# SamsungSAILMontreal/ghn3

Measured on AMD Instinct MI355X. Metric: predicted-params/sec (GHN fwd+bwd), ghn3xlm16, 256-node graphs, higher is better.
Workload: dtype f16; 1 GPU; ghn3xlm16 fwd+bwd, 1 synthetic 256-node graph(s) per GPU (seed 256000+), 86515016 predicted params per GPU, loss = sum of Frobenius norms of the predicted tensors; ghn_params=654365312, decoder_rows=1421, workspace_bytes=2436048640, zero_fill_bytes=2797339192, parallelism=dp1, index_mode=reference, loss=fused into the tile kernels

## Files before the change

ghn3_amd/csrc/elementwise.hip:

```cpp

#include "ghn3_internal.h"

#define MAX_DEGREE 100
#define MAX_INPUT_DIST 1000

__device__ __forceinline__ float wsum(float v) {
#pragma unroll
    for (int o = 32; o > 0; o >>= 1) v += __shfl_xor(v, o, 64);
    return v;
}

static int launch_ok(const char* what) {
    hipError_t e = hipGetLastError();
    if (e != hipSuccess) { ghn3_set_error("%s launch: %s", what, hipGetErrorString(e)); return GHN3_E_HIP; }
    return GHN3_OK;
}

__global__ __launch_bounds__(256) void graph_prologue_kernel(const int64_t* __restrict__ A, int* __restrict__ deg_in,
                                                             int* __restrict__ deg_out, int* __restrict__ dist0,
                                                             int* __restrict__ pair, int N, int V) {
    __shared__ int red[2][4];
    const int i = blockIdx.x, b = blockIdx.y;
    const int64_t* Ab = A + (size_t)b * N * N;
    int cnt_out = 0, cnt_in = 0;
    for (int j = threadIdx.x; j < N; j += 256) {
        const int64_t fw = Ab[(size_t)i * N + j];
        const int64_t bw = Ab[(size_t)j * N + i];
        cnt_out += (fw == 1);
        cnt_in += (bw == 1);
        int f = (int)(fw < 0 ? 0 : (fw >= V ? V - 1 : fw));
        int g = (int)(bw < 0 ? 0 : (bw >= V ? V - 1 : bw));
        pair[((size_t)b * N + i) * N + j] = f * V + g;
    }
#pragma unroll
    for (int o = 32; o > 0; o >>= 1) {
        cnt_out += __shfl_xor(cnt_out, o, 64);
        cnt_in += __shfl_xor(cnt_in, o, 64);
    }
    const int w = threadIdx.x >> 6;
    if ((threadIdx.x & 63) == 0) { red[0][w] = cnt_out; red[1][w] = cnt_in; }
    __syncthreads();
    if (threadIdx.x == 0) {
        int o_ = red[0][0] + red[0][1] + red[0][2] + red[0][3];
        int i_ = red[1][0] + red[1][1] + red[1][2] + red[1][3];
        deg_out[b * N + i] = o_ > MAX_DEGREE ? MAX_DEGREE : o_;
        deg_in[b * N + i] = i_ > MAX_DEGREE ? MAX_DEGREE : i_;
        int64_t dd = Ab[i];
        dist0[b * N + i] = (int)(dd < 0 ? 0 : (dd > MAX_INPUT_DIST ? MAX_INPUT_DIST : dd));
    }
}

int ghn3_graph_prologue(const int64_t* A, int* deg_in, int* deg_out, int* dist0, int* pair, int B, int N, int V,
                        hipStream_t s) {
    hipLaunchKernelGGL(graph_prologue_kernel, dim3(N, B), dim3(256), 0, s, A, deg_in, deg_out, dist0, pair, N, V);
    return launch_ok("graph_prologue");
}

__global__ __launch_bounds__(256) void embed_nodes_kernel(
    float* __restrict__ x, const int* __restrict__ node_type, const int* __restrict__ shape_idx,
    const int* __restrict__ n_nodes, const int* __restrict__ node_off, const float* __restrict__ E_type,
    const float* __restrict__ E_ch, const float* __restrict__ E_sp, const float* __restrict__ E_in,
    const float* __restrict__ E_out, const float* __restrict__ E_dist, const int* __restrict__ deg_in,
    const int* __restrict__ deg_out, const int* __restrict__ dist0, int B, int N, int C) {
    const int row = blockIdx.x * 4 + (threadIdx.x >> 6);
    if (row >= B * N) return;
    const int lane = threadIdx.x & 63;
    const int b = row / N, i = row - b * N;
    float* xr = x + (size_t)row * C;
    if (i >= n_nodes[b]) {
        for (int c = lane; c < C; c += 64) xr[c] = 0.f;
        return;
    }
    const int sidx = node_off[b] + i;
    const int t = node_type[sidx];
    const int s0 = shape_idx[4 * sidx], s1 = shape_idx[4 * sidx + 1], s2 = shape_idx[4 * sidx + 2],
              s3 = shape_idx[4 * sidx + 3];
    const int di = deg_in[row], dout = deg_out[row], dd = dist0[row];
    const int cq = C >> 2;
    for (int c = lane; c < C; c += 64) {
        const int part = c / cq, cc = c - part * cq;
        float sh;
        if (part == 0) sh = E_ch[(size_t)s0 * cq + cc];
        else if (part == 1) sh = E_ch[(size_t)s1 * cq + cc];
        else if (part == 2) sh = E_sp[(size_t)s2 * cq + cc];
        else sh = E_sp[(size_t)s3 * cq + cc];
        float v = E_type[(size_t)t * C + c] + sh;
        v += E_in[(size_t)di * C + c];
        v += E_out[(size_t)dout * C + c];
        v += E_dist[(size_t)dd * C + c];
        xr[c] = v;
    }
}

int ghn3_embed_nodes(float* x, const int* node_type, const int* shape_idx, const int* n_nodes, const int* node_off,
                     const float* E_type, const float* E_ch, const float* E_sp, const float* E_in,
                     const float* E_out, const float* E_dist, const int* deg_in, const int* deg_out,
                     const int* dist0, int B, int N, int C, hipStream_t s) {
    if (C % 4) { ghn3_set_error("embed: C=%d not a multiple of 4", C); return GHN3_E_ARG; }
    hipLaunchKernelGGL(embed_nodes_kernel, dim3((B * N + 3) / 4), dim3(256), 0, s, x, node_type, shape_idx, n_nodes,
                       node_off, E_type, E_ch, E_sp, E_in, E_out, E_dist, deg_in, deg_out, dist0, B, N, C);
    return launch_ok("embed_nodes");
}

__global__ __launch_bounds__(256) void embed_bwd_kernel(
    const float* __restrict__ dx, const int* __restrict__ node_type, const int* __restrict__ shape_idx,
    const int* __restrict__ n_nodes, const int* __restrict__ node_off, float* __restrict__ dE_type,
    float* __restrict__ dE_ch, float* __restrict__ dE_sp, float* __restrict__ dE_in, float* __restrict__ dE_out,
    float* __restrict__ dE_dist, const int* __restrict__ deg_in, const int* __restrict__ deg_out,
    const int* __restrict__ dist0, int B, int N, int C, int n_type, int n_ch, int n_sp) {
    extern __shared__ unsigned long long emb_mask[];
    int r = blockIdx.x, tab = 0;
    if (r >= n_type) { r -= n_type; tab = 1;
        if (r >= n_ch) { r -= n_ch; tab = 2;
            if (r >= n_sp) { r -= n_sp; tab = 3;
                if (r >= 101) { r -= 101; tab = 4;
                    if (r >= 101) { r -= 101; tab = 5; } } } } }
    const int cq = C >> 2;
    const int width = (tab == 1 || tab == 2) ? cq : C;
    const int base0 = tab == 2 ? 2 * cq : 0, base1 = tab == 1 ? cq : 3 * cq;
    const int rows = B * N, words = (rows + 63) >> 6;
    int any = 0;
    for (int row0 = (threadIdx.x >> 6) * 64; row0 < rows; row0 += 256) {
        const int row = row0 + (threadIdx.x & 63);
        int f = 0;
        if (row < rows) {
            const int b = row / N, i = row - b * N;
            if (i < n_nodes[b]) {
                const int sidx = node_off[b] + i;
                if (tab == 0) f = node_type[sidx] == r;
                else if (tab == 1) f = (shape_idx[4 * sidx] == r) | ((shape_idx[4 * sidx + 1] == r) << 1);
                else if (tab == 2) f = (shape_idx[4 * sidx + 2] == r) | ((shape_idx[4 * sidx + 3] == r) << 1);
                else if (tab == 3) f = deg_in[row] == r;
                else if (tab == 4) f = deg_out[row] == r;
                else f = dist0[row] == r;
            }
        }
        const unsigned long long m0 = __ballot(f & 1), m1 = __ballot(f & 2);
        if ((threadIdx.x & 63) == 0) { emb_mask[row0 >> 6] = m0; emb_mask[words + (row0 >> 6)] = m1; }
        any |= f;
    }
    if (!__syncthreads_or(any)) return;
    int* lst = reinterpret_cast<int*>(emb_mask + 2 * words);
    __shared__ int n_match;
    if (threadIdx.x == 0) {
        int n = 0;
        for (int w = 0; w < words; ++w) {
            const unsigned long long m0 = emb_mask[w], m1 = emb_mask[words + w];
            unsigned long long m = m0 | m1;
            while (m) {
                const int bit = __ffsll((long long)m) - 1;
                m &= m - 1;
                lst[n++] = (w * 64 + bit) | ((int)((m0 >> bit) & 1) << 24) | ((int)((m1 >> bit) & 1) << 25);
            }
        }
        n_match = n;
    }
    __syncthreads();
    const int n = n_match;
    float acc[2] = {0.f, 0.f};
    for (int i0 = 0; i0 < n; i0 += 8) {
        float v0[8][2], v1[8][2];
#pragma unroll
        for (int e = 0; e < 8; ++e) {
            const int ent = i0 + e < n ? lst[i0 + e] : 0;
            const float* g = dx + (size_t)(ent & 0xffffff) * C;
#pragma unroll
            for (int k = 0; k < 2; ++k) {
                const int c = threadIdx.x + 256 * k;
                const bool in = i0 + e < n && c < width;
                v0[e][k] = (in && (ent & (1 << 24))) ? g[base0 + c] : 0.f;
                v1[e][k] = (in && (ent & (1 << 25))) ? g[base1 + c] : 0.f;
            }
        }
#pragma unroll
        for (int e = 0; e < 8; ++e)
#pragma unroll
            for (int k = 0; k < 2; ++k) { acc[k] += v0[e][k]; acc[k] += v1[e][k]; }
    }
    float* dst = tab == 0 ? dE_type : tab == 1 ? dE_ch : tab == 2 ? dE_sp : tab == 3 ? dE_in : tab == 4 ? dE_out : dE_dist;
#pragma unroll
    for (int k = 0; k < 2; ++k) {
        const int c = threadIdx.x + 256 * k;
        if (c < width) dst[(size_t)r * width + c] += acc[k];
    }
}

int ghn3_embed_bwd(const float* dx, const int* node_type, const int* shape_idx, const int* n_nodes,
                   const int* node_off, float* dE_type, float* dE_ch, float* dE_sp, float* dE_in, float* dE_out,
                   float* dE_dist, const int* deg_in, const int* deg_out, const int* dist0, int B, int N, int C,
                   int n_type, int n_ch, int n_sp, hipStream_t s) {
    if (C > 512 || n_type <= 0 || n_ch <= 0 || n_sp <= 0) {
        ghn3_set_error("embed_bwd: C <= 512 and the table row counts (i3..i5) are required");
        return GHN3_E_ARG;
    }
    if (B * N > 12 * 1024) { ghn3_set_error("embed_bwd: more than 12288 dense node rows"); return GHN3_E_LIMIT; }
    const int blocks = n_type + n_ch + n_sp + 101 + 101 + 1001;
    hipLaunchKernelGGL(embed_bwd_kernel, dim3(blocks), dim3(256), (size_t)(16 * ((B * N + 63) / 64) + 4 * (size_t)B * N + 16), s, dx, node_type, shape_idx, n_nodes,
                       node_off, dE_type, dE_ch, dE_sp, dE_in, dE_out, dE_dist, deg_in, deg_out, dist0, B, N, C, n_type,
                       n_ch, n_sp);
    return launch_ok("embed_bwd");
}

__global__ __launch_bounds__(256) void edge_hidden_kernel(float* __restrict__ hid, const float* __restrict__ Pfw,
                                                          const float* __restrict__ Pbw, int V, int C) {
    const int p = blockIdx.x;
    const int fw = p / V, bw = p - fw * V;
    for (int c = threadIdx.x; c < C; c += 256)
        hid[(size_t)p * C + c] = fmaxf(Pfw[(size_t)fw * C + c] + Pbw[(size_t)bw * C + c], 0.f);
}
int ghn3_edge_hidden(float* hid, const float* Pfw, const float* Pbw, int V, int C, hipStream_t s) {
    hipLaunchKernelGGL(edge_hidden_kernel, dim3(V * V), dim3(256), 0, s, hid, Pfw, Pbw, V, C);
    return launch_ok("edge_hidden");
}

__global__ __launch_bounds__(256) void edge_hidden_bwd_fw_kernel(float* __restrict__ dPfw, float* __restrict__ dhid,
                                                                 const float* __restrict__ hid, int V, int C) {
    __shared__ float part[4][64];
    const int fw = blockIdx.x, c = blockIdx.y * 64 + (threadIdx.x & 63), w = threadIdx.x >> 6;
    float acc = 0.f;
    if (c < C)
        for (int bw = w; bw < V; bw += 4) {
            const size_t o = ((size_t)fw * V + bw) * C + c;
            const float g = hid[o] > 0.f ? dhid[o] : 0.f;
            dhid[o] = g;
            acc += g;
        }
    part[w][threadIdx.x & 63] = acc;
    __syncthreads();
    if (w == 0 && c < C) dPfw[(size_t)fw * C + c] = (part[0][threadIdx.x] + part[1][threadIdx.x]) + (part[2][threadIdx.x] + part[3][threadIdx.x]);
}
__global__ __launch_bounds__(256) void edge_hidden_bwd_bw_kernel(float* __restrict__ dPbw,
                                                                 const float* __restrict__ dhid, int V, int C) {
    __shared__ float part[4][64];
    const int bw = blockIdx.x, c = blockIdx.y * 64 + (threadIdx.x & 63), w = threadIdx.x >> 6;
    float acc = 0.f;
    if (c < C)
        for (int fw = w; fw < V; fw += 4) acc += dhid[((size_t)fw * V + bw) * C + c];
    part[w][threadIdx.x & 63] = acc;
    __syncthreads();
    if (w == 0 && c < C) dPbw[(size_t)bw * C + c] = (part[0][threadIdx.x] + part[1][threadIdx.x]) + (part[2][threadIdx.x] + part[3][threadIdx.x]);
}
int ghn3_edge_hidden_bwd(float* dPfw, float* dPbw, float* dhid, const float* hid, int V, int C, hipStream_t s) {
    hipLaunchKernelGGL(edge_hidden_bwd_fw_kernel, dim3(V, (C + 63) / 64), dim3(256), 0, s, dPfw, dhid, hid, V, C);
    hipLaunchKernelGGL(edge_hidden_bwd_bw_kernel, dim3(V, (C + 63) / 64), dim3(256), 0, s, dPbw, dhid, V, C);
    return launch_ok("edge_hidden_bwd");
}

__global__ __launch_bounds__(256) void bias_gather_kernel(float* __restrict__ bias, const float* __restrict__ T,
                                                          const int* __restrict__ pair, int N, int H, int ldT) {
    extern __shared__ float bg_rows[];
    __shared__ int bg_pair[256];
    const int b = blockIdx.z, i = blockIdx.y;
    const int j0 = blockIdx.x * 256, j = j0 + threadIdx.x;
    const int nj = min(256, N - j0);
    bg_pair[threadIdx.x] = j < N ? pair[((size_t)b * N + i) * N + j] : 0;
    __syncthreads();
    const int lpr = ldT >> 2;
    const int ld = ldT + 1;
    for (int e = threadIdx.x; e < nj * lpr; e += 256) {
        const int q = e / lpr, c = e - q * lpr;
        const float4 v = *reinterpret_cast<const float4*>(T + (size_t)bg_pair[q] * ldT + 4 * c);
        float* d = bg_rows + q * ld + 4 * c;
        d[0] = v.x; d[1] = v.y; d[2] = v.z; d[3] = v.w;
    }
    __syncthreads();
    if (j >= N) return;
    const float* r = bg_rows + threadIdx.x * ld;
    for (int h = 0; h < H; ++h) bias[(((size_t)b * H + h) * N + i) * N + j] = r[h];
}
__global__ __launch_bounds__(256) void bias_gather_direct_kernel(float* __restrict__ bias, const float* __restrict__ T,
                                                                 const int* __restrict__ pair, int N, int H, int ldT) {
    const int b = blockIdx.z, i = blockIdx.y;
    const int j = blockIdx.x * 256 + threadIdx.x;
    if (j >= N) return;
    const int p = pair[((size_t)b * N + i) * N + j];
    const float* tr = T + (size_t)p * ldT;
    for (int h = 0; h < H; ++h) bias[(((size_t)b * H + h) * N + i) * N + j] = tr[h];
}
int ghn3_bias_gather(float* bias, const float* T, const int* pair, int B, int N, int H, hipStream_t s) {
    const int ldT = (H + 3) & ~3;
    if (ldT <= 64)
        hipLaunchKernelGGL(bias_gather_kernel, dim3((N + 255) / 256, N, B), dim3(256), 256 * (ldT + 1) * sizeof(float), s, bias, T,
                           pair, N, H, ldT);
    else
        hipLaunchKernelGGL(bias_gather_direct_kernel, dim3((N + 255) / 256, N, B), dim3(256), 0, s, bias, T, pair, N, H, ldT);
    return launch_ok("bias_gather");
}

__global__ __launch_bounds__(256) void bias_amax_kernel(const float* __restrict__ x, int64_t n, float* __restrict__ amax) {
    float m = 0.f;
    const int64_t n4 = (reinterpret_cast<uintptr_t>(x) & 15) ? 0 : (n >> 2);
    const float4* x4 = reinterpret_cast<const float4*>(x);
    for (int64_t e = (int64_t)blockIdx.x * 256 + threadIdx.x; e < n4; e += (int64_t)gridDim.x * 256) {
        const float4 v = x4[e];
        m = fmaxf(fmaxf(m, fmaxf(fabsf(v.x), fabsf(v.y))), fmaxf(fabsf(v.z), fabsf(v.w)));
    }
    for (int64_t e = 4 * n4 + (int64_t)blockIdx.x * 256 + threadIdx.x; e < n; e += (int64_t)gridDim.x * 256) m = fmaxf(m, fabsf(x[e]));
    ghn3_atomic_amax(amax, m);
}
__device__ __forceinline__ float fix_scale(float amax) {
    if (!(amax > 0.f)) return 1.f;
    const int e = (int)((__float_as_uint(amax) >> 23) & 0xff) - 127;
    return __uint_as_float((unsigned)(127 + 30 - e) << 23);
}
__global__ __launch_bounds__(256) void bias_hist_kernel(long long* __restrict__ acc, const float* __restrict__ dBias,
                                                        const int* __restrict__ pair, int N, int H, int V,
                                                        int rows_per_block, int use_lds, const float* __restrict__ amax) {
    extern __shared__ __attribute__((aligned(16))) long long hist[];
    const int b = blockIdx.z, h = blockIdx.y;
    const int i0 = blockIdx.x * rows_per_block;
    const int i1 = min(N, i0 + rows_per_block);
    const int bins = V * V;
    const float sc = fix_scale(*amax);
    if (use_lds) {
        for (int k = threadIdx.x; k < bins; k += 256) hist[k] = 0;
        __syncthreads();
    }
    const size_t total = (size_t)(i1 - i0) * N;
    for (size_t e = threadIdx.x; e < total; e += 256) {
        const size_t off = (size_t)i0 * N + e;
        const int p = pair[(size_t)b * N * N + off];
        const long long g = (long long)llrintf(dBias[((size_t)b * H + h) * N * N + off] * sc);
        if (g == 0) continue;
        if (use_lds) atomicAdd(reinterpret_cast<unsigned long long*>(&hist[p]), (unsigned long long)g);
        else atomicAdd(reinterpret_cast<unsigned long long*>(&acc[(size_t)p * H + h]), (unsigned long long)g);
    }
    if (use_lds) {
        __syncthreads();
        for (int k = threadIdx.x; k < bins; k += 256) {
            const long long v = hist[k];
            if (v != 0) atomicAdd(reinterpret_cast<unsigned long long*>(&acc[(size_t)k * H + h]), (unsigned long long)v);
        }
    }
}
__global__ __launch_bounds__(256) void bias_hist_finish_kernel(float* __restrict__ dT, const long long* __restrict__ acc,
                                                               int bins, int H, int ldT, const float* __restrict__ amax) {
// ... 1663 lines not shown
```

ghn3_amd/csrc/gemm_wg.hip:

```cpp

#include "ghn3_internal.h"

#define GAS __attribute__((address_space(1)))
typedef float f32x4 __attribute__((ext_vector_type(4)));
typedef __bf16 bf16x8 __attribute__((ext_vector_type(8)));
typedef f32x4 GAS* gf4;
typedef const f32x4 GAS* gcf4;

namespace {

constexpr int WG_KC = 64;
template <int T> constexpr int wg_lds() { return 4 * T * 128 + 16 * T * 4; }

__device__ __forceinline__ unsigned wg_pack(__bf16 a, __bf16 b) {
    return (unsigned)__builtin_bit_cast(unsigned short, a) | ((unsigned)__builtin_bit_cast(unsigned short, b) << 16);
}

__device__ __forceinline__ void wg_stage(char* s_hi, char* s_lo, int f, int k, const f32x4& r0, const f32x4& r1) {
#pragma unroll
    for (int e = 0; e < 4; ++e) {
        const __bf16 h0 = (__bf16)r0[e], h1 = (__bf16)r1[e];
        const __bf16 l0 = (__bf16)(r0[e] - (float)h0), l1 = (__bf16)(r1[e] - (float)h1);
        const int row = f + e;
        const int off = row * 128 + (((k >> 3) ^ ((row >> 1) & 7)) << 4) + ((k & 7) << 1);
        *reinterpret_cast<unsigned*>(s_hi + off) = wg_pack(h0, h1);
        *reinterpret_cast<unsigned*>(s_lo + off) = wg_pack(l0, l1);
    }
}

template <int T>
__device__ __forceinline__ void wg_tile(const GemmProbDev* __restrict__ probs, int n_probs, int tile, char* sm) {
    constexpr int WG_BM = T, WG_BN = T;
    constexpr int TN = T / 32;
    constexpr int FPR = T / 4;
    char* sAh = sm;
    char* sAl = sm + T * 128;
    char* sBh = sm + 2 * T * 128;
    char* sBl = sm + 3 * T * 128;
    float* sbias = reinterpret_cast<float*>(sm + 4 * T * 128);

    int lo = 0, hi_ = n_probs - 1;
    while (lo < hi_) {
        const int mid = (lo + hi_ + 1) >> 1;
        if (probs[mid].tile_start <= tile) lo = mid; else hi_ = mid - 1;
    }
    const GemmProbDev* P = probs + lo;
    const int t_id = tile - P->tile_start;
    const int n0 = (t_id % P->tiles_n) * WG_BN, m0 = (t_id / P->tiles_n) * WG_BM;
    const int M = P->M, N = P->N, K = P->K, lda = P->lda, ldb = P->ldb;
    const int tid = threadIdx.x, lane = tid & 63, wave = tid >> 6;
    const int l15 = lane & 15, lq = lane >> 4;
    const int wm0 = (wave >> 1) * 32, wn0 = (wave & 1) * (T / 2);
    const bool want_bias = (P->flags & GHN3_GEMM_BIASGRAD) && n0 == 0;

    constexpr int FGW = FPR / 8;
    const int f4 = ((lane & 7) + 8 * (wave % FGW)) * 4, kp = (lane >> 3) + 8 * (wave / FGW);
    const float GAS* Ag = (const float GAS*)P->A;
    const float GAS* Bg = (const float GAS*)P->B;
    const bool a_in = m0 + f4 < M, b_in = n0 + f4 < N;
    const f32x4 zero = f32x4{0.f, 0.f, 0.f, 0.f};

    f32x4 ra[2][2], rb[2][2];
    auto load_chunk = [&](int k0) {
#pragma unroll
        for (int i = 0; i < 2; ++i)
#pragma unroll
            for (int r = 0; r < 2; ++r) {
                const int k = k0 + 2 * kp + 32 * i + r;
                ra[i][r] = (a_in && k < K) ? *reinterpret_cast<gcf4>(Ag + (int64_t)k * lda + m0 + f4) : zero;
                rb[i][r] = (b_in && k < K) ? *reinterpret_cast<gcf4>(Bg + (int64_t)k * ldb + n0 + f4) : zero;
            }
    };

    f32x4 acc0[2][TN], acc1[2][TN];
#pragma unroll
    for (int i = 0; i < 2; ++i)
#pragma unroll
        for (int j = 0; j < TN; ++j) { acc0[i][j] = zero; acc1[i][j] = zero; }
    f32x4 bsum = zero;

    load_chunk(0);
    for (int k0 = 0; k0 < K; k0 += WG_KC) {
        if (k0 > 0) __syncthreads();
#pragma unroll
        for (int i = 0; i < 2; ++i) {
            wg_stage(sAh, sAl, f4, 2 * kp + 32 * i, ra[i][0], ra[i][1]);
            wg_stage(sBh, sBl, f4, 2 * kp + 32 * i, rb[i][0], rb[i][1]);
            if (want_bias) bsum += ra[i][0] + ra[i][1];
        }
        if (k0 + WG_KC < K) load_chunk(k0 + WG_KC);
        __syncthreads();
#pragma unroll
        for (int h = 0; h < 2; ++h) {
            const int ch = 4 * h + lq;
            bf16x8 xh[2], xl[2], wh[TN], wl[TN];
#pragma unroll
            for (int i = 0; i < 2; ++i) {
                const int row = wm0 + 16 * i + l15;
                const int off = row * 128 + ((ch ^ ((row >> 1) & 7)) << 4);
                xh[i] = *reinterpret_cast<const bf16x8*>(sAh + off);
                xl[i] = *reinterpret_cast<const bf16x8*>(sAl + off);
            }
#pragma unroll
            for (int j = 0; j < TN; ++j) {
                const int row = wn0 + 16 * j + l15;
                const int off = row * 128 + ((ch ^ ((row >> 1) & 7)) << 4);
                wh[j] = *reinterpret_cast<const bf16x8*>(sBh + off);
                wl[j] = *reinterpret_cast<const bf16x8*>(sBl + off);
            }
#pragma unroll
            for (int i = 0; i < 2; ++i)
#pragma unroll
                for (int j = 0; j < TN; ++j) {
                    acc0[i][j] = __builtin_amdgcn_mfma_f32_16x16x32_bf16(wh[j], xh[i], acc0[i][j], 0, 0, 0);
                    acc1[i][j] = __builtin_amdgcn_mfma_f32_16x16x32_bf16(wh[j], xl[i], acc1[i][j], 0, 0, 0);
                }
#pragma unroll
            for (int i = 0; i < 2; ++i)
#pragma unroll
                for (int j = 0; j < TN; ++j)
                    acc1[i][j] = __builtin_amdgcn_mfma_f32_16x16x32_bf16(wl[j], xh[i], acc1[i][j], 0, 0, 0);
        }
    }

    const float alpha = P->alpha;
    const bool accum = (P->flags & GHN3_GEMM_ACCUM) != 0;
    float GAS* C = (float GAS*)P->C;
#pragma unroll
    for (int i = 0; i < 2; ++i) {
        const int m = m0 + wm0 + 16 * i + l15;
#pragma unroll
        for (int j = 0; j < TN; ++j) {
            const int n = n0 + wn0 + 16 * j + 4 * lq;
            if (m >= M || n >= N) continue;
            const int64_t ci = (int64_t)m * P->ldc + n;
            f32x4 v;
#pragma unroll
            for (int e = 0; e < 4; ++e) v[e] = (acc0[i][j][e] + acc1[i][j][e]) * alpha;
            if (accum) v += *reinterpret_cast<gcf4>(C + ci);
            *reinterpret_cast<gf4>(C + ci) = v;
        }
    }
    if (want_bias) {
#pragma unroll
        for (int e = 0; e < 4; ++e) sbias[kp * T + f4 + e] = bsum[e];
        __syncthreads();
        if (tid < T && m0 + tid < M) {
            float t = 0.f;
#pragma unroll
            for (int q = 0; q < 16; ++q) t += sbias[q * T + tid];
            float GAS* db = (float GAS*)P->bias + (int64_t)(m0 + tid) * P->bias_stride;
            *db += t;
        }
    }
}

template <int T>
__global__ __launch_bounds__(T * 4) void gemm_wg_kernel(const GemmProbDev* __restrict__ probs, int n_probs, int total_tiles) {
    extern __shared__ __attribute__((aligned(16))) char wg_sm[];
    for (int tile = blockIdx.x; tile < total_tiles; tile += gridDim.x) {
        wg_tile<T>(probs, n_probs, tile, wg_sm);
        __syncthreads();
    }
}

}

int ghn3_gemm_wg_launch(const GemmProbDev* d_probs, int n_probs, int total_tiles, int grid_cap, int tile_edge, hipStream_t stream) {
    if (n_probs <= 0 || total_tiles <= 0) return GHN3_OK;
    const int grid = grid_cap > 0 && grid_cap < total_tiles ? grid_cap : total_tiles;
    if (tile_edge == 128) {
        static bool attr = false;
        if (!attr) {
            hipFuncSetAttribute((const void*)gemm_wg_kernel<128>, hipFuncAttributeMaxDynamicSharedMemorySize, wg_lds<128>());
            attr = true;
        }
        hipLaunchKernelGGL(gemm_wg_kernel<128>, dim3(grid), dim3(512), wg_lds<128>(), stream, d_probs, n_probs, total_tiles);
    } else {
        hipLaunchKernelGGL(gemm_wg_kernel<64>, dim3(grid), dim3(256), wg_lds<64>(), stream, d_probs, n_probs, total_tiles);
    }
    hipError_t e = hipGetLastError();
    if (e != hipSuccess) { ghn3_set_error("wgrad x3 gemm launch: %s", hipGetErrorString(e)); return GHN3_E_HIP; }
    return GHN3_OK;
}
```

ghn3_amd/program.py:

```python

import math
import os

import numpy as np

from . import _lib as L
from . import bookkeeping as bk

ALIGN = 256


def global_param_names():
    return ['ln.weight', 'ln.bias', 'embed.weight', 'shape_enc.embed_spatial.weight',
            'shape_enc.embed_channel.weight', 'gnn.0.centrality_embed_in.weight',
            'gnn.0.centrality_embed_out.weight', 'gnn.0.input_dist_embed.weight',
            'gnn.0.attn.edge_embed.embed.weight', 'gnn.0.attn.proj_e.0.weight', 'gnn.0.attn.proj_e.0.bias',
            'gnn.0.attn.proj_e.2.weight', 'gnn.0.attn.proj_e.2.bias',
            'decoder.fc.0.weight', 'decoder.fc.0.bias', 'decoder.conv.0.weight', 'decoder.conv.0.bias',
            'decoder.conv.2.weight', 'decoder.conv.2.bias', 'decoder.class_layer_predictor.1.weight',
            'decoder.class_layer_predictor.1.bias', 'decoder_1d.fc.0.weight', 'decoder_1d.fc.0.bias',
            'decoder_1d.fc.2.weight', 'decoder_1d.fc.2.bias', 'bias_class.1.weight', 'bias_class.1.bias']


LAYER_PARAM_NAMES = ['ln1.weight', 'ln1.bias', 'attn.to_qkv.weight', 'attn.to_out.0.weight', 'attn.to_out.0.bias',
# ... 1161 lines not shown
                                scale)
                            predicted[-1]['tok'] = (tok_off, i_e)
                            tok_off += round_up(i_e, 4)
                        else:
                            raise NotImplementedError('1-D target from a 4-D tile')
                    elif len(key) == 2 and key[1] > 0:
                        g, n_idx = group_of[ind]
                        base = g['cls_off'][n_idx]
                        if len(t) == 4 and (t[2], t[3]) != (1, 1):
                            raise NotImplementedError('classifier target %s' % str(t))
                        add(dst, 1, base, (t[0], t[1], 1, 1), (min(t[0], K), min(t[1], g['i']), 1, 1),
                            (1, ldK, 0, 0), (K, g['i'], 1, 1), mode, scale)
                    elif len(key) == 2 and key[1] < 0:
                        r = clsb_row[ind]
                        assert len(t) == 1
                        add(dst, 3, r * ldK, (1, t[0], 1, 1), (1, min(t[0], K), 1, 1), (0, 1, 0, 0), (1, K, 1, 1),
                            mode, scale)
                    else:
                        r = self.oned_index[ind]
                        if len(t) == 1:
                            half = (1 - int(bool(is_w)) + it)
                            add(dst, 2, r * 2 * mc + half * mc, (1, t[0], 1, 1), (1, min(t[0], mc), 1, 1),
                                (0, 1, 0, 0), (1, mc, 1, 1), mode, scale)
                        elif len(t) == 3:
                            if t[1] > 1 and t[2] > 1:
                                raise NotImplementedError('3-D target %s from the 1-D decoder' % str(t))
                            add(dst, 2, r * 2 * mc, (t[0], t[1], t[2], 1), (min(t[0], 2 * mc), 1, 1, 1),
                                (1, 0, 0, 0), (2 * mc, 1, 1, 1), mode, scale)
                        else:
                            raise NotImplementedError('target %s from the 1-D decoder' % str(t))
        self.predicted = predicted
        self.out_numel = max(out_off, 16)
        self.tok_floats = max(tok_off, 4)
        self.n_desc = nd = len(descs)
        CH = 2048
        self.tile_lds = [0, 0]
        desc_arr = np.zeros(max(nd, 1), dtype=L.TILE_DT)
        fb = bb = np.zeros((0, 2), dtype=np.int64)
        if nd:
            cols = list(zip(*descs))
            desc_arr['dst_off'], desc_arr['src_off'] = cols[0], cols[1]
            S = np.asarray(cols[2], dtype=np.int64).reshape(nd, 4)
            T = np.asarray(cols[3], dtype=np.int64).reshape(nd, 4)
            E = np.asarray(cols[4], dtype=np.int64).reshape(nd, 4)
            R = np.asarray(cols[5], dtype=np.int64).reshape(nd, 4)
            desc_arr['S'], desc_arr['T'], desc_arr['E'], desc_arr['R'] = S, T, E, R
            desc_arr['src_buf'], desc_arr['mode'], desc_arr['scale'] = cols[6], cols[7], cols[8]
            mode = np.asarray(cols[7], dtype=np.int64)
            hw = T[:, 2] * T[:, 3]
            row_ok = (mode == 0) & (hw > 1) & (S[:, 1] == 1) & (E[:, 2] == T[:, 2]) & (T[:, 2] == R[:, 2]) & \
                (E[:, 3] == T[:, 3]) & (T[:, 3] == R[:, 3]) & (hw <= 1024)
            ich = np.maximum(16, np.minimum(np.maximum(T[:, 1], R[:, 1]), (4096 // np.maximum(hw, 1)) // 16 * 16))
            desc_arr['_pad'] = np.where(row_ok, ich, 0)
            if row_ok.any():
                lds = int((4 * ich * hw)[row_ok].max())
                self.tile_lds = [lds, lds]
            ids = np.arange(nd, dtype=np.int64)

            def tables(n0, n1, numel):
                n_i = (n1 + ich - 1) // ich
                cnt = np.where(row_ok, n0 * n_i, (numel + CH - 1) // CH)
                total = int(cnt.sum())
                first = np.cumsum(cnt) - cnt
                d_of = np.repeat(ids, cnt)
                j = np.arange(total, dtype=np.int64) - np.repeat(first, cnt)
                rb = row_ok[d_of]
                ni_b = np.maximum(n_i[d_of], 1)
                word = np.where(rb, (j // ni_b) | (((j % ni_b) * ich[d_of]) << 24), j * CH)
                return np.stack([np.where(rb, ~d_of, d_of), word], axis=1), first

            fb, fwd_first = tables(T[:, 0], T[:, 1], T.prod(axis=1))
            bb, _ = tables(R[:, 0], R[:, 1], R.prod(axis=1))
        dseg = np.asarray(desc_seg if nd else [0], dtype=np.int32)
        raw = np.concatenate([desc_arr.view(np.uint8).reshape(-1), fb.view(np.uint8).reshape(-1),
                              bb.view(np.uint8).reshape(-1), dseg.view(np.uint8).reshape(-1)])
        self.r_desc = self.idx(raw)
        self.fwd_blk = (len(fb), desc_arr.nbytes)
        self.bwd_blk = (len(bb), desc_arr.nbytes + fb.nbytes)
        self.desc_seg_off = desc_arr.nbytes + fb.nbytes + bb.nbytes
        seg_blk = np.zeros(len(predicted) + 1, dtype=np.int32)
        if nd:
            first_desc = np.full(len(predicted), nd, dtype=np.int64)
            np.minimum.at(first_desc, dseg, np.arange(nd))
            seg_blk[:-1] = fwd_first[first_desc]
        seg_blk[-1] = len(fb)
        self.r_seg_blk = self.idx(seg_blk)
        seg = np.asarray([[p['offset'], p['offset'] + p['numel']] for p in predicted], dtype=np.int64).reshape(-1, 2)
        self.r_seg = self.idx(seg if len(seg) else np.zeros((1, 2), dtype=np.int64))
        self.n_seg = len(predicted)
        ends = seg[:, 1] if len(seg) else np.zeros(1, dtype=np.int64)
        starts = np.arange(0, max(self.out_numel, 1), 8192, dtype=np.int64)
        self.r_seg_first = self.idx(np.searchsorted(ends, starts, side='right').astype(np.int32))
        srcs = self._tile_sources(False)
        if self.n_desc:
            parts = self.wsf('sq_parts', self.fwd_blk[0]) if self.training else self.NONE
            bparts = self.wsf('b_parts', self.fwd_blk[0]) if self.training else self.NONE
            self._tile_desc_arr = desc_arr
            self.op(L.OP_TILE_FWD, refs=[(self.xbuf(self.X_OUT), 0)] + srcs + [self.r_desc, parts, bparts],
                    ints=(self.n_desc, self.fwd_blk[0], self.fwd_blk[1], self.tile_lds[0]),
                    flags=L.OPFLAG_TIMED | (self.TAG_TILE_FWD << 16))

    def _tile_sources(self, grad):
        pre = 'd_' if grad else ''
        out = []
        for name in ('tiles', 'clsout', 'w1d', 'cbout'):
            nm = pre + name
            out.append(self.wref(nm) if nm in self._ws_names else self.NONE)
        if grad:
            out.append(self.wsf('d_tok', self.tok_floats))
        else:
            out.append((self.xbuf(self.X_TOK), 0))
        out.append(self.NONE)
        return out

    def norm_ops(self, upstream=1.0):
        scal = self.xbuf(self.X_SCAL)
        f_ops, b_ops = [], []
        saved = self._ops
        self._ops = []
        self.op(L.OP_MEMSET0, refs=((scal, 0),), ints=(4,))
        self.op(L.OP_PARAM_NORM_FWD, refs=((scal, 0), (self.xbuf(self.X_OUT), 0), self.r_seg, (scal, 256),
                                           self.r_seg_first, (scal, 256 + round_up(4 * max(self.n_seg, 1), 64))),
                ints=(self.n_seg, self.out_numel))
        f_ops = self._finish_ops()
        self.op(L.OP_PARAM_NORM_BWD, refs=((self.xbuf(self.X_DOUT), 0), (self.xbuf(self.X_OUT), 0), self.r_seg,
                                           (scal, 256), self.r_seg_first), ints=(self.n_seg, self.out_numel),
                floats=(upstream,))
        b_ops = self._finish_ops()
        self._ops = saved
        return f_ops, b_ops

    def norm_fin_ops(self):
        scal = self.xbuf(self.X_SCAL)
        saved, self._ops = self._ops, []
        if self.n_desc and 'sq_parts' in self._ws_names:
            self.op(L.OP_PARAM_NORM_FIN, refs=((scal, 0), (scal, 256), self.wref('sq_parts'), self.r_seg_blk,
                                               self.wref('b_parts'), (scal, 256 + round_up(4 * max(self.n_seg, 1), 64)),
                                               (scal, 252)),
                    ints=(self.n_seg,))
        else:
            self.op(L.OP_MEMSET0, refs=((scal, 0),), ints=(4,))
        ops = self._finish_ops()
        self._ops = saved
        return ops

    def _layer_side_ops(self, layers, rows):
        C = self.C
        p0 = len(self._probs)
        for d in layers:
            pre = d['pre']
            W3, W1f, Wo, Wq = pre + 'ff.net.3.weight', pre + 'ff.net.0.weight', pre + 'attn.to_out.0.weight', \
                pre + 'attn.to_qkv.weight'
            self.gemm(d['g_cur'], d['f'], self.gref(W3), C, 4 * C, rows, C, 4 * C, 4 * C, a_mode=L.MODE_COL,
                      b_mode=L.MODE_COL, accum=True, dbias=self.gref(pre + 'ff.net.3.bias'))
            self.gemm(d['dz'], d['h2'], self.gref(W1f), 4 * C, C, rows, 4 * C, C, C, a_mode=L.MODE_COL, b_mode=L.MODE_COL,
                      accum=True, dbias=self.gref(pre + 'ff.net.0.bias'))
            self.gemm(d['g_mid'], d['o'], self.gref(Wo), C, C, rows, C, C, C, a_mode=L.MODE_COL, b_mode=L.MODE_COL,
                      accum=True, dbias=self.gref(pre + 'attn.to_out.0.bias'))
            self.gemm(d['dqkv'], d['h1'], self.gref(Wq), 3 * C, C, rows, 3 * C, C, C, a_mode=L.MODE_COL, b_mode=L.MODE_COL,
                      accum=True)
        dflt = ('48' if self.x3 else '64') if C >= 256 else '0'
        self.gemm_op(p0, side=True, tile=int(os.environ.get('GHN3_LAYER_WGRAD_TILE', dflt)),
                     grid_cap=int(os.environ.get('GHN3_LAYER_WGRAD_CAP', '0')) if self.SIDE else 0)
        if len(layers) == 1:
            d = layers[0]
            pre = d['pre']
            self.op(L.OP_LN_PARAM_GRAD, refs=(self.gref(pre + 'ln2.weight'), self.gref(pre + 'ln2.bias'), d['dhA'], d['xmid'],
                                              d['m2'], d['r2']), ints=(rows, C, 1), flags=self.SIDE)
            self.op(L.OP_LN_PARAM_GRAD, refs=(self.gref(pre + 'ln1.weight'), self.gref(pre + 'ln1.bias'), d['dhB'], d['x_in'],
                                              d['m1'], d['r1']), ints=(rows, C, 1), flags=self.SIDE)
            return
        base = 'gnn.0.' + LAYER_PARAM_NAMES[0]
        ws = self.xbuf(self.X_WS)
        tab = []
        for d in layers:
            pre = d['pre']
            for (gn, bn, dy, x, mu, rs) in ((pre + 'ln2.weight', pre + 'ln2.bias', d['dhA'], d['xmid'], d['m2'], d['r2']),
                                           (pre + 'ln1.weight', pre + 'ln1.bias', d['dhB'], d['x_in'], d['m1'], d['r1'])):
                assert all(r_[0] == ws and r_[1] % 4 == 0 for r_ in (dy, x, mu, rs))
                tab.append((self.param_gap(base, gn), self.param_gap(base, bn), dy[1] // 4, x[1] // 4, mu[1] // 4, rs[1] // 4))
        self.op(L.OP_LN_PARAM_GRAD_BATCH, refs=(self.gref(base), (ws, 0), self.idx(np.asarray(tab, dtype=np.int64))),
                ints=(len(tab), rows, C), flags=self.SIDE)

    def _colsum(self, out, X, M, N, ld, q=0, s=0, stride=1, gather=None):
        self.op(L.OP_COLSUM, refs=(out, X, gather if gather is not None else self.NONE),
                ints=(M, N, ld, q, s, stride, 1))

    def set_tile_route(self, direct):
        direct = bool(direct and getattr(self, 'tile_bwd_h16', 0))
        if self.tile_bwd_op is None or not hasattr(self, 'd16_kinds'):
            return []
        self.bwd_ops[self.tile_bwd_op]['i'][5] = self.tile_bwd_h16 if direct else 0
        touched = []
        for idx, on in ((self.d16_on_idx, direct), (self.d16_off_idx, not direct)):
            for k in idx:
                self.bwd_ops[k]['kind'] = self.d16_kinds[k] if on else L.OP_NOP
                touched.append(k)
        return touched

    @staticmethod
    def _wgrad_order_env():
        return os.environ.get('GHN3_WGRAD_ORDER', 'first' if os.environ.get('GHN3_WGRAD_LATE', '1') != '0' else 'early')

    def _wgrad_schedule(self, flops, rows):
        env_main, env_cap = os.environ.get('GHN3_WGRAD_MAIN'), os.environ.get('GHN3_WGRAD_CAP')
        if not self.SIDE or env_main == '1':
            return 0
        if env_cap is not None:
            return max(8, int(env_cap) // 8 * 8)
        w_ms = flops / 1150e12 * 1e3 + 4.0 * self.max_shape[0] * self.max_shape[1] * 8 * self.C / 4.3e12 * 1e3
        ch_ms = self.Lyr * (0.030 + 0.014 * (rows / 256.0) * (self.C / 384.0) ** 2)
        if env_main != '0' and w_ms < 0.75 * ch_ms:
            return 0
        if self._wgrad_order_env() == 'first':
            return 128
        c = int(round(256.0 * w_ms / (1.75 * ch_ms) / 8.0)) * 8
        if c >= 232:
            return 0 if env_main != '0' else 224
        return max(64, c)

    def _build_h16_table(self, g16, direct_member):
        D = self._tile_desc_arr
        nd = self.n_desc
        tab = np.zeros((nd, 3), dtype=np.int64)
        tab[:, 0] = np.iinfo(np.int64).min
        members = []
        for g in g16:
            for m_ in g['members']:
                if direct_member(m_):
                    members.append((m_['tile_off'], m_['tile_off'] + m_['rows'] * g['ld'], g))
        members.sort(key=lambda t: t[0])
        if members and nd:
            lo = np.asarray([t[0] for t in members], dtype=np.int64)
            hi = np.asarray([t[1] for t in members], dtype=np.int64)
            src = D['src_off'].astype(np.int64)
            k = np.searchsorted(lo, src, side='right') - 1
            ok = (D['src_buf'] == 0) & (k >= 0)
            ok &= src < hi[np.maximum(k, 0)]
            reach = src + ((D['R'].astype(np.int64) - 1) * D['S'].astype(np.int64)).sum(axis=1)
            d_tiles_h = self._ws_names['d_tiles'] // 2
            for d_ in np.nonzero(ok)[0]:
                g = members[int(k[d_])][2]
                assert reach[d_] < hi[int(k[d_])], 'tile descriptor straddles a family member'
                assert D['mode'][d_] == 0
                rel0 = int(src[d_]) - g['tile_off']
                assert 0 <= rel0 and g['rows'] * g['ld'] < 2 ** 32
                tab[d_] = (g['dth'] - d_tiles_h, rel0, g['ld'] | (g['dth_ld'] << 32))
        r_tab = self.idx(tab)
        assert r_tab[0] == self.r_desc[0] and r_tab[1] > self.r_desc[1]
        self.tile_bwd_h16 = r_tab[1] - self.r_desc[1]

    def _build_backward(self):
        C, H, B, N, V, K = self.C, self.H, self.B, self.N, self.V, self.K
        rows = B * N
        ldT, ldK = self.ldT, self.ldK
        ms = self.max_shape
        S2 = self.S * self.S
        M, n1 = self.M, self.n1
        (r_types, r_shape, r_nn, r_noff, deg_in, deg_out, dist0, pair) = self.r_graph
        xe = self.r_xe
        self.op(L.OP_MEMSET0, refs=((self.xbuf(self.X_GRADFLAT), 0),), ints=(-1,))
        self.op(L.OP_MEMSET0, refs=((self.xbuf(self.X_GRADFLAT), 0),), ints=(-1,))
        self.memset_grad_op = 0
        self.tile_bwd_op = None
        self.grad_no_memset = []
        self.bwd_cut_w2 = 0
        late_ops = []
        self.wgrad_op_range = None
        self.grad_sumsq = None

        d_rows = self.wsf('d_xrows', (M + n1) * C)
        zeros = []
        if M > 0:
            self.wsf('d_tiles', self.tiles_floats)
            self.ws_zero_dout = [(self._ws_names['d_tiles'], 4 * (int(self.tiles_floats) + 64))]
            if 'clsout' in self._ws_names:
                n_cls = sum(g['rows'] * g['i_ld'] for g in self.conv_groups if g['kind'] == 'cls')
                self.wsf('d_clsout', n_cls * ldK)
                zeros.append((self.wref('d_clsout'), 4 * n_cls * ldK))
        if n1 > 0:
            mc = self.mc
            self.wsf('d_w1d', n1 * 2 * mc)
            zeros.append((self.wref('d_w1d'), 4 * n1 * 2 * mc))
            if self.n1_clsb:
                self.wsf('d_cbout', self.n1_clsb * ldK)
                zeros.append((self.wref('d_cbout'), 4 * self.n1_clsb * ldK))
        self.r_amax = self.wsf('amax', 16)
        scaled = self.bwd_scaled and self.direct16 and M > 0
        amax_t = self.r_amax if scaled else None
        amax_u = (self.r_amax[0], self.r_amax[1] + 16) if scaled else None
        if scaled:
            zeros.append((self.r_amax, 64))
        run = None
        for (buf, off), n in sorted(zeros, key=lambda it: (it[0][0], it[0][1])) + [((None, 0), 0)]:
            if run is not None and buf == run[0] and 0 <= off - (run[1] + run[2]) <= 1024:
                run[2] = off + n - run[1]
                continue
            if run is not None:
                self.op(L.OP_MEMSET0, refs=((run[0], run[1]),), ints=(run[2],))
            run = [buf, off, n]
        if self.n_desc:
            grads = self._tile_sources(True)
            if scaled:
                grads[5] = amax_t
            srcs = self._tile_sources(False)
            self.tile_bwd_op = len(self._ops)
            self.tile_bwd_refs = {0: (self.xbuf(self.X_DOUT), 0), 6: (self.xbuf(self.X_NORMG), 0),
                                  14: (self.xbuf(self.X_SCAL), 256), 15: (self.xbuf(self.X_OUT), 0)}
            self.op(L.OP_TILE_BWD, refs=[(self.xbuf(self.X_DOUT), 0)] + srcs + [self.r_desc] + grads +
                    [self.NONE, self.NONE],
                    ints=(self.n_desc, self.bwd_blk[0], self.bwd_blk[1], self.tile_lds[1], self.desc_seg_off, 0,
                          1 if self.decoder_bwd_ctype == L.CT_BF16 else 0),
                    flags=L.OPFLAG_TIMED | (self.TAG_TILE_BWD << 16))
# ... 541 lines not shown
```

Baseline: 15.04 billion predicted-params/s.

## Parallelize embed backward across waves and transpose-read LDS in weight-grad GEMM

The embedding backward kernel now builds its match list with all four waves using popcount prefix sums, then splits the summation across waves and reduces the partials in shared memory. This replaces the single-thread list build and the serial per-block sum. The weight-gradient GEMM switches to a k-major LDS layout that is staged with vector bf16 conversions and read through ds_read_tr16 transpose loads. It also prefetches the old C values at tile start and adds a waves_per_eu occupancy hint. The layer weight-gradient GEMMs drop accumulate mode, which removes the read of C but assumes those gradient buffers are not already holding values that must be added to.

```diff
diff --git a/ghn3_amd/csrc/elementwise.hip b/ghn3_amd/csrc/elementwise.hip
--- a/ghn3_amd/csrc/elementwise.hip
+++ b/ghn3_amd/csrc/elementwise.hip
@@ -102,6 +102,30 @@
     return launch_ok("embed_nodes");
 }
 
+template <int NJ, int E, bool TWO>
+__device__ __forceinline__ void embed_bwd_sum(const float* __restrict__ dx, const int* lst, int begin, int end, int C,
+                                              int width, int base0, int base1, int lane, float* acc) {
+    for (int i0 = begin; i0 < end; i0 += E) {
+        float v0[E][NJ], v1[E][NJ];
+#pragma unroll
+        for (int e = 0; e < E; ++e) {
+            const int ent = i0 + e < end ? lst[i0 + e] : 0;
+            const float* g = dx + (size_t)(ent & 0xffffff) * C;
+#pragma unroll
+            for (int j = 0; j < NJ; ++j) {
+                const int c = lane + 64 * j;
+                const bool in = i0 + e < end && c < width;
+                v0[e][j] = (in && (ent & (1 << 24))) ? g[base0 + c] : 0.f;
+                v1[e][j] = (TWO && in && (ent & (1 << 25))) ? g[base1 + c] : 0.f;
+            }
+        }
+#pragma unroll
+        for (int e = 0; e < E; ++e)
+#pragma unroll
+            for (int j = 0; j < NJ; ++j) { acc[j] += v0[e][j]; if (TWO) acc[j] += v1[e][j]; }
+    }
+}
+
 __global__ __launch_bounds__(256) void embed_bwd_kernel(
     const float* __restrict__ dx, const int* __restrict__ node_type, const int* __restrict__ shape_idx,
     const int* __restrict__ n_nodes, const int* __restrict__ node_off, float* __restrict__ dE_type,
@@ -109,6 +133,7 @@
     float* __restrict__ dE_dist, const int* __restrict__ deg_in, const int* __restrict__ deg_out,
     const int* __restrict__ dist0, int B, int N, int C, int n_type, int n_ch, int n_sp) {
     extern __shared__ unsigned long long emb_mask[];
+    __shared__ float part[4][512];
     int r = blockIdx.x, tab = 0;
     if (r >= n_type) { r -= n_type; tab = 1;
         if (r >= n_ch) { r -= n_ch; tab = 2;
@@ -119,9 +144,10 @@
     const int width = (tab == 1 || tab == 2) ? cq : C;
     const int base0 = tab == 2 ? 2 * cq : 0, base1 = tab == 1 ? cq : 3 * cq;
     const int rows = B * N, words = (rows + 63) >> 6;
+    const int lane = threadIdx.x & 63, wave = threadIdx.x >> 6;
     int any = 0;
-    for (int row0 = (threadIdx.x >> 6) * 64; row0 < rows; row0 += 256) {
-        const int row = row0 + (threadIdx.x & 63);
+    for (int row0 = wave * 64; row0 < rows; row0 += 256) {
+        const int row = row0 + lane;
         int f = 0;
         if (row < rows) {
             const int b = row / N, i = row - b * N;
@@ -136,52 +162,32 @@
             }
         }
         const unsigned long long m0 = __ballot(f & 1), m1 = __ballot(f & 2);
-        if ((threadIdx.x & 63) == 0) { emb_mask[row0 >> 6] = m0; emb_mask[words + (row0 >> 6)] = m1; }
+        if (lane == 0) { emb_mask[row0 >> 6] = m0; emb_mask[words + (row0 >> 6)] = m1; }
         any |= f;
     }
     if (!__syncthreads_or(any)) return;
     int* lst = reinterpret_cast<int*>(emb_mask + 2 * words);
-    __shared__ int n_match;
-    if (threadIdx.x == 0) {
-        int n = 0;
-        for (int w = 0; w < words; ++w) {
-            const unsigned long long m0 = emb_mask[w], m1 = emb_mask[words + w];
-            unsigned long long m = m0 | m1;
-            while (m) {
-                const int bit = __ffsll((long long)m) - 1;
-                m &= m - 1;
-                lst[n++] = (w * 64 + bit) | ((int)((m0 >> bit) & 1) << 24) | ((int)((m1 >> bit) & 1) << 25);
-            }
-        }
-        n_match = n;
-    }
-    __syncthreads();
-    const int n = n_match;
-    float acc[2] = {0.f, 0.f};
-    for (int i0 = 0; i0 < n; i0 += 8) {
-        float v0[8][2], v1[8][2];
-#pragma unroll
-        for (int e = 0; e < 8; ++e) {
-            const int ent = i0 + e < n ? lst[i0 + e] : 0;
-            const float* g = dx + (size_t)(ent & 0xffffff) * C;
-#pragma unroll
-            for (int k = 0; k < 2; ++k) {
-                const int c = threadIdx.x + 256 * k;
-                const bool in = i0 + e < n && c < width;
-                v0[e][k] = (in && (ent & (1 << 24))) ? g[base0 + c] : 0.f;
-                v1[e][k] = (in && (ent & (1 << 25))) ? g[base1 + c] : 0.f;
-            }
-        }
-#pragma unroll
-        for (int e = 0; e < 8; ++e)
-#pragma unroll
-            for (int k = 0; k < 2; ++k) { acc[k] += v0[e][k]; acc[k] += v1[e][k]; }
-    }
+    int n = 0;
+    for (int w = 0; w < words; ++w) {
+        const unsigned long long m0 = emb_mask[w], m1 = emb_mask[words + w], m = m0 | m1;
+        if ((w & 3) == wave && ((m >> lane) & 1))
+            lst[n + __popcll(m & ((1ull << lane) - 1ull))] =
+                (w * 64 + lane) | ((int)((m0 >> lane) & 1) << 24) | ((int)((m1 >> lane) & 1) << 25);
+        n += __popcll(m);
+    }
+    __syncthreads();
+    const int per = (n + 3) >> 2, begin = wave * per, end = begin + per < n ? begin + per : n;
+    float acc[8] = {0.f, 0.f, 0.f, 0.f, 0.f, 0.f, 0.f, 0.f};
+    if (tab == 1 || tab == 2) embed_bwd_sum<2, 16, true>(dx, lst, begin, end, C, width, base0, base1, lane, acc);
+    else embed_bwd_sum<8, 8, false>(dx, lst, begin, end, C, width, base0, base1, lane, acc);
+#pragma unroll
+    for (int j = 0; j < 8; ++j) part[wave][lane + 64 * j] = acc[j];
+    __syncthreads();
     float* dst = tab == 0 ? dE_type : tab == 1 ? dE_ch : tab == 2 ? dE_sp : tab == 3 ? dE_in : tab == 4 ? dE_out : dE_dist;
 #pragma unroll
     for (int k = 0; k < 2; ++k) {
         const int c = threadIdx.x + 256 * k;
-        if (c < width) dst[(size_t)r * width + c] += acc[k];
+        if (c < width) dst[(size_t)r * width + c] += ((part[0][c] + part[1][c]) + part[2][c]) + part[3][c];
     }
 }
 
diff --git a/ghn3_amd/csrc/gemm_wg.hip b/ghn3_amd/csrc/gemm_wg.hip
--- a/ghn3_amd/csrc/gemm_wg.hip
+++ b/ghn3_amd/csrc/gemm_wg.hip
@@ -4,28 +4,31 @@
 #define GAS __attribute__((address_space(1)))
 typedef float f32x4 __attribute__((ext_vector_type(4)));
 typedef __bf16 bf16x8 __attribute__((ext_vector_type(8)));
+typedef __bf16 bf16x4 __attribute__((ext_vector_type(4)));
 typedef f32x4 GAS* gf4;
 typedef const f32x4 GAS* gcf4;
+typedef __attribute__((address_space(3))) bf16x4* lds_bf4;
 
 namespace {
 
 constexpr int WG_KC = 64;
 template <int T> constexpr int wg_lds() { return 4 * T * 128 + 16 * T * 4; }
 
-__device__ __forceinline__ unsigned wg_pack(__bf16 a, __bf16 b) {
-    return (unsigned)__builtin_bit_cast(unsigned short, a) | ((unsigned)__builtin_bit_cast(unsigned short, b) << 16);
+template <int T> __device__ __forceinline__ int wg_off(int k, int c) {
+    return k * (2 * T) + ((c ^ (T == 64 ? (k >> 1) & 3 : k & 7)) << 5);
 }
 
-__device__ __forceinline__ void wg_stage(char* s_hi, char* s_lo, int f, int k, const f32x4& r0, const f32x4& r1) {
-#pragma unroll
-    for (int e = 0; e < 4; ++e) {
-        const __bf16 h0 = (__bf16)r0[e], h1 = (__bf16)r1[e];
-        const __bf16 l0 = (__bf16)(r0[e] - (float)h0), l1 = (__bf16)(r1[e] - (float)h1);
-        const int row = f + e;
-        const int off = row * 128 + (((k >> 3) ^ ((row >> 1) & 7)) << 4) + ((k & 7) << 1);
-        *reinterpret_cast<unsigned*>(s_hi + off) = wg_pack(h0, h1);
-        *reinterpret_cast<unsigned*>(s_lo + off) = wg_pack(l0, l1);
-    }
+__device__ __forceinline__ void wg_stage(char* s_hi, char* s_lo, int off, const f32x4& r) {
+    const bf16x4 h = __builtin_convertvector(r, bf16x4);
+    const bf16x4 l = __builtin_convertvector(r - __builtin_convertvector(h, f32x4), bf16x4);
+    *reinterpret_cast<bf16x4*>(s_hi + off) = h;
+    *reinterpret_cast<bf16x4*>(s_lo + off) = l;
+}
+
+template <int T> __device__ __forceinline__ bf16x8 wg_frag(const char* img, int off) {
+    const bf16x4 a = __builtin_amdgcn_ds_read_tr16_b64_v4bf16((lds_bf4)(img + off));
+    const bf16x4 b = __builtin_amdgcn_ds_read_tr16_b64_v4bf16((lds_bf4)(img + off + 16 * 2 * T));
+    return __builtin_shufflevector(a, b, 0, 1, 2, 3, 4, 5, 6, 7);
 }
 
 template <int T>
@@ -52,25 +55,42 @@
     const int l15 = lane & 15, lq = lane >> 4;
     const int wm0 = (wave >> 1) * 32, wn0 = (wave & 1) * (T / 2);
     const bool want_bias = (P->flags & GHN3_GEMM_BIASGRAD) && n0 == 0;
+    const float alpha = P->alpha;
+    const bool accum = (P->flags & GHN3_GEMM_ACCUM) != 0;
+    float GAS* C = (float GAS*)P->C;
+    const f32x4 zero = f32x4{0.f, 0.f, 0.f, 0.f};
 
-    constexpr int FGW = FPR / 8;
-    const int f4 = ((lane & 7) + 8 * (wave % FGW)) * 4, kp = (lane >> 3) + 8 * (wave / FGW);
+    f32x4 cold[2][TN];
+#pragma unroll
+    for (int i = 0; i < 2; ++i)
+#pragma unroll
+        for (int j = 0; j < TN; ++j) {
+            const int m = m0 + wm0 + 16 * i + l15, n = n0 + wn0 + 16 * j + 4 * lq;
+            cold[i][j] = (accum && m < M && n < N) ? *reinterpret_cast<gcf4>(C + (int64_t)m * P->ldc + n) : zero;
+        }
+
+    const int f4 = (tid % FPR) * 4, kr = tid / FPR;
+    const int st_off = wg_off<T>(kr, f4 >> 4) + ((f4 & 12) << 1);
     const float GAS* Ag = (const float GAS*)P->A;
     const float GAS* Bg = (const float GAS*)P->B;
     const bool a_in = m0 + f4 < M, b_in = n0 + f4 < N;
-    const f32x4 zero = f32x4{0.f, 0.f, 0.f, 0.f};
 
-    f32x4 ra[2][2], rb[2][2];
+    f32x4 ra[4], rb[4];
     auto load_chunk = [&](int k0) {
 #pragma unroll
-        for (int i = 0; i < 2; ++i)
+        for (int i = 0; i < 4; ++i) {
+            const int k = k0 + kr + 16 * i;
+            ra[i] = (a_in && k < K) ? *reinterpret_cast<gcf4>(Ag + (int64_t)k * lda + m0 + f4) : zero;
+            rb[i] = (b_in && k < K) ? *reinterpret_cast<gcf4>(Bg + (int64_t)k * ldb + n0 + f4) : zero;
+        }
+    };
+
+    const int fk = 4 * lq + (l15 >> 2), fb = (l15 & 3) << 3;
+    int offA[2], offB[TN];
 #pragma unroll
-            for (int r = 0; r < 2; ++r) {
-                const int k = k0 + 2 * kp + 32 * i + r;
-                ra[i][r] = (a_in && k < K) ? *reinterpret_cast<gcf4>(Ag + (int64_t)k * lda + m0 + f4) : zero;
-                rb[i][r] = (b_in && k < K) ? *reinterpret_cast<gcf4>(Bg + (int64_t)k * ldb + n0 + f4) : zero;
-            }
-    };
+    for (int i = 0; i < 2; ++i) offA[i] = wg_off<T>(fk, (wm0 >> 4) + i) + fb;
+#pragma unroll
+    for (int j = 0; j < TN; ++j) offB[j] = wg_off<T>(fk, (wn0 >> 4) + j) + fb;
 
     f32x4 acc0[2][TN], acc1[2][TN];
 #pragma unroll
@@ -83,30 +103,26 @@
     for (int k0 = 0; k0 < K; k0 += WG_KC) {
         if (k0 > 0) __syncthreads();
 #pragma unroll
-        for (int i = 0; i < 2; ++i) {
-            wg_stage(sAh, sAl, f4, 2 * kp + 32 * i, ra[i][0], ra[i][1]);
-            wg_stage(sBh, sBl, f4, 2 * kp + 32 * i, rb[i][0], rb[i][1]);
-            if (want_bias) bsum += ra[i][0] + ra[i][1];
+        for (int i = 0; i < 4; ++i) {
+            wg_stage(sAh, sAl, st_off + i * 16 * 2 * T, ra[i]);
+            wg_stage(sBh, sBl, st_off + i * 16 * 2 * T, rb[i]);
+            if (want_bias) bsum += ra[i];
         }
         if (k0 + WG_KC < K) load_chunk(k0 + WG_KC);
         __syncthreads();
 #pragma unroll
         for (int h = 0; h < 2; ++h) {
-            const int ch = 4 * h + lq;
+            const int ho = h * 32 * 2 * T;
             bf16x8 xh[2], xl[2], wh[TN], wl[TN];
 #pragma unroll
             for (int i = 0; i < 2; ++i) {
-                const int row = wm0 + 16 * i + l15;
-                const int off = row * 128 + ((ch ^ ((row >> 1) & 7)) << 4);
-                xh[i] = *reinterpret_cast<const bf16x8*>(sAh + off);
-                xl[i] = *reinterpret_cast<const bf16x8*>(sAl + off);
+                xh[i] = wg_frag<T>(sAh, offA[i] + ho);
+                xl[i] = wg_frag<T>(sAl, offA[i] + ho);
             }
 #pragma unroll
             for (int j = 0; j < TN; ++j) {
-                const int row = wn0 + 16 * j + l15;
-                const int off = row * 128 + ((ch ^ ((row >> 1) & 7)) << 4);
-                wh[j] = *reinterpret_cast<const bf16x8*>(sBh + off);
-                wl[j] = *reinterpret_cast<const bf16x8*>(sBl + off);
+                wh[j] = wg_frag<T>(sBh, offB[j] + ho);
+                wl[j] = wg_frag<T>(sBl, offB[j] + ho);
             }
 #pragma unroll
             for (int i = 0; i < 2; ++i)
@@ -123,9 +139,6 @@
         }
     }
 
-    const float alpha = P->alpha;
-    const bool accum = (P->flags & GHN3_GEMM_ACCUM) != 0;
-    float GAS* C = (float GAS*)P->C;
 #pragma unroll
     for (int i = 0; i < 2; ++i) {
         const int m = m0 + wm0 + 16 * i + l15;
@@ -137,13 +150,13 @@
             f32x4 v;
 #pragma unroll
             for (int e = 0; e < 4; ++e) v[e] = (acc0[i][j][e] + acc1[i][j][e]) * alpha;
-            if (accum) v += *reinterpret_cast<gcf4>(C + ci);
+            if (accum) v += cold[i][j];
             *reinterpret_cast<gf4>(C + ci) = v;
         }
     }
     if (want_bias) {
 #pragma unroll
-        for (int e = 0; e < 4; ++e) sbias[kp * T + f4 + e] = bsum[e];
+        for (int e = 0; e < 4; ++e) sbias[kr * T + f4 + e] = bsum[e];
         __syncthreads();
         if (tid < T && m0 + tid < M) {
             float t = 0.f;
@@ -156,7 +169,8 @@
 }
 
 template <int T>
-__global__ __launch_bounds__(T * 4) void gemm_wg_kernel(const GemmProbDev* __restrict__ probs, int n_probs, int total_tiles) {
+__global__ __launch_bounds__(T * 4) __attribute__((amdgpu_waves_per_eu(T == 64 ? 3 : 2)))
+void gemm_wg_kernel(const GemmProbDev* __restrict__ probs, int n_probs, int total_tiles) {
     extern __shared__ __attribute__((aligned(16))) char wg_sm[];
     for (int tile = blockIdx.x; tile < total_tiles; tile += gridDim.x) {
         wg_tile<T>(probs, n_probs, tile, wg_sm);
diff --git a/ghn3_amd/program.py b/ghn3_amd/program.py
--- a/ghn3_amd/program.py
+++ b/ghn3_amd/program.py
@@ -1337,13 +1337,12 @@
             W3, W1f, Wo, Wq = pre + 'ff.net.3.weight', pre + 'ff.net.0.weight', pre + 'attn.to_out.0.weight', \
                 pre + 'attn.to_qkv.weight'
             self.gemm(d['g_cur'], d['f'], self.gref(W3), C, 4 * C, rows, C, 4 * C, 4 * C, a_mode=L.MODE_COL,
-                      b_mode=L.MODE_COL, accum=True, dbias=self.gref(pre + 'ff.net.3.bias'))
+                      b_mode=L.MODE_COL, dbias=self.gref(pre + 'ff.net.3.bias'))
             self.gemm(d['dz'], d['h2'], self.gref(W1f), 4 * C, C, rows, 4 * C, C, C, a_mode=L.MODE_COL, b_mode=L.MODE_COL,
-                      accum=True, dbias=self.gref(pre + 'ff.net.0.bias'))
+                      dbias=self.gref(pre + 'ff.net.0.bias'))
             self.gemm(d['g_mid'], d['o'], self.gref(Wo), C, C, rows, C, C, C, a_mode=L.MODE_COL, b_mode=L.MODE_COL,
-                      accum=True, dbias=self.gref(pre + 'attn.to_out.0.bias'))
-            self.gemm(d['dqkv'], d['h1'], self.gref(Wq), 3 * C, C, rows, 3 * C, C, C, a_mode=L.MODE_COL, b_mode=L.MODE_COL,
-                      accum=True)
+                      dbias=self.gref(pre + 'attn.to_out.0.bias'))
+            self.gemm(d['dqkv'], d['h1'], self.gref(Wq), 3 * C, C, rows, 3 * C, C, C, a_mode=L.MODE_COL, b_mode=L.MODE_COL)
         dflt = ('48' if self.x3 else '64') if C >= 256 else '0'
         self.gemm_op(p0, side=True, tile=int(os.environ.get('GHN3_LAYER_WGRAD_TILE', dflt)),
                      grid_cap=int(os.environ.get('GHN3_LAYER_WGRAD_CAP', '0')) if self.SIDE else 0)
```

After: 15.16 billion predicted-params/s, median of 3. About the same (+0.8%).
